# santiagolmedo/gnn_qot_estimation

Measured on AMD Instinct MI355X. Metric: graphs/sec (train step) on 100-node/400-edge synthetic topologies, batch=1024, higher is better.
Workload: dtype f32; 1 GPU; configs[1]: 2-layer TopologicalGNN (TransformerConv+NNConv) hidden=64, 100-node/400-directed-edge topologies, batch=1024 graphs per GPU, dropout 0.5, SGD momentum 0.9, SmoothL1; CSR build included in every step; graphs_per_gpu=1024, global_batch=1024, distinct_graphs_per_gpu=1024, launch=hip-graph replay, 4 whole steps (fwd+bwd+optimizer each) per graph, steps_per_graph=4, collective_in_graph=False, parallelism=dp1, prime_steps=45, collective_world_size=1, all_reduce_floats=68715

## Files before the change

gnn_qot_estimation_amd/_lib.py:

```python
from __future__ import annotations

import ctypes as C
import os
import subprocess

import torch

_HERE = os.path.dirname(os.path.abspath(__file__))
LIB_PATH = os.environ.get("QOT_LIB_PATH") or os.path.join(_HERE, "libqot_gnn.so")
CSRC_DIR = os.path.join(_HERE, "csrc")

_p = C.c_void_p
_i64 = C.c_int64
_int = C.c_int
_f = C.c_float
_u64 = C.c_uint64
_sz = C.c_size_t

ABI_VERSION = 13

_INFER_COMMON = ([_p] * 5 + [_i64] * 3 + [_int, _int, _p, _int, _p, _int, _p, _int] + [_p] * 9
                 + [_f, _f, _p, _int, _int, _int, _p])
_LP_COMMON = ([_p] * 6 + [_i64] * 4 + [_p] * 4 + [_f] + [_p] * 4 + [_f] + [_p] * 4 + [_f, _p, _p] + [_int] * 5 + [_p])

# ... 122 lines not shown
                                      _i64, _i64, _i64, _i64, _i64, _p, _p, _p, _p, _p, _p, _p, _p, _p]),
    "qot_shard_stage_gather": (_int, [_p, _i64, _p, _p, _p, _p, _i64, _i64, _i64, _p, _p, _int, _p, _p, _int, _p, _int, _i64,
                                      _i64, _i64, _i64, _i64, _i64, _p, _p, _p, _p, _p, _p, _p, _p, _p]),
    "qot_gather3": (_int, [_p, _i64, _p, _i64, _p, _p, _p, _i64, _p]),
    "qot_gemm_nt": (_int, [_p, _i64, _p, _i64, _p, _i64, _i64, _int, _int, _p, _p, _p, _p]),
    "qot_gemm_nt_planes": (_int, [_p, _i64, _p, _i64, _p, _i64, _int, _int, _int, _p]),
    "qot_gemm_tn_splits": (_int, [_int, _int, _i64]),
    "qot_gemm256_takes": (_int, [_i64, _int]),
    "qot_gemm_tn_planes": (_int, [_p, _i64, _p, _i64, _p, _int, _int, _i64, _int, _p, _p, _p]),
    "qot_skinny_linear_fwd": (_int, [_p, _p, _p, _i64, _int, _int, _p]),
    "qot_skinny_linear_fwd_logits": (_int, [_p, _p, _p, _i64, _int, _int, _p, _p, _p, _p, _p]),
    "qot_gemm_nt_logits": (_int, [_p, _i64, _p, _i64, _p, _i64, _i64, _int, _int, _p, _p, _p, _p, _p, _p, _p, _p]),
    "qot_skinny_linear_dw_blocks": (_int, [_i64]),
    "qot_skinny_linear_dw": (_int, [_p, _p, _p, _i64, _int, _int, _p]),
    "qot_run_roles": (_int, [_p, _int, _p]),
    "qot_rows_gather": (_int, [_p, _p, _p, _i64, _int, _p]),
    "qot_rows_scatter": (_int, [_p, _p, _p, _i64, _int, _p]),
    **{f"qot_topological_infer{k}_supported": (_int, [_int] * 5) for k in ("", "_mc", "_grad", "_whatif")},
    **{f"qot_topological_infer{k}_max_edges": (_int, [_int] * 3) for k in ("", "_mc", "_grad", "_whatif")},
    "qot_topological_infer": (_int, _INFER_COMMON + [_p]),
    "qot_topological_infer_mc": (_int, _INFER_COMMON + [_int, _i64, _u64, _f, _f, _int, _p]),
    "qot_topological_infer_grad": (_int, _INFER_COMMON + [_p, _int, _p, _p, _p]),
    "qot_topological_infer_whatif": (_int, _INFER_COMMON + [_p, _p, _p, _i64, _p, _p, _i64, _p, _i64, _int, _p]),
    "qot_lightpath_infer": (_int, _LP_COMMON + [_p]),
    "qot_lightpath_infer_grad": (_int, _LP_COMMON + [_p, _int, _p, _p, _p, _p, _p]),
    "qot_lightpath_infer_whatif": (_int, _LP_COMMON + [_p, _p, _p, _i64, _p, _p, _i64, _i64, _p]),
    "qot_status_graph_scratch_bytes": (_sz, [_i64, _i64, _i64, _int]),
    "qot_status_graph_count": (_int, [_p, _p, _p, _i64, _i64, _int, _i64, _i64, _int, _int, _int, C.c_double, _int, _p, _sz, _p,
                                      _p]),
    "qot_status_graph_fill": (_int, [_p, _p, _p, _i64, _i64, _int, _i64, _i64, _int, _int, _int, _int, _p, _int, _p, _int, _p,
                                     _p, _p, _p, _i64, _i64, _p, _p, _p, _p, _p]),
}

MAX_ROLES = 12
(ROLE_CSR_BY_GRAPH, ROLE_TABLE_PROJECT_FWD, ROLE_GATHER3, ROLE_SUM_ROWS, ROLE_NNCONV_FINALIZE64, ROLE_TABLE_PROJECT_BWD,
 ROLE_TABLE_SCORES, ROLE_TABLE_PROJECT_BWD_SCORES) = range(1, 9)


class Role(C.Structure):
    _fields_ = [("kind", C.c_int32), ("reserved", C.c_int32), ("p", C.c_void_p * 18), ("i", C.c_int64 * 8)]


def make_role(kind: int, ptrs, ints) -> Role:
    r = Role()
    r.kind = kind
    for k, t in enumerate(ptrs):
        r.p[k] = None if t is None else (t.data_ptr() if isinstance(t, torch.Tensor) else int(t))
    for k, v in enumerate(ints):
        r.i[k] = int(v)
    return r


def run_roles(roles, stream_handle=None):
    if not roles:
        return
    if len(roles) > MAX_ROLES:
        for k in range(0, len(roles), MAX_ROLES):
            run_roles(roles[k:k + MAX_ROLES], stream_handle)
        return
    arr = (Role * len(roles))(*roles)
    code = (_lib or load()).qot_run_roles(C.addressof(arr), len(roles), stream() if stream_handle is None else stream_handle)
    if code != 0:
        check(code, "qot_run_roles")


_lib = None


class QotError(RuntimeError):
    """A libqot_gnn entry point returned a non-zero status."""


def build_library(verbose: bool = False) -> str:
    cmd = ["make", "-C", CSRC_DIR, "-j", str(min(8, os.cpu_count() or 1))]
    res = subprocess.run(cmd, capture_output=True, text=True)
    if res.returncode != 0:
        raise RuntimeError("building libqot_gnn.so failed:\n" + res.stdout[-4000:] + res.stderr[-8000:])
    if verbose:
# ... 19 lines not shown
        raise QotError(f"libqot_gnn ABI version {lib.qot_abi_version()} != {ABI_VERSION} expected by this package: "
                       "rebuild with `make -C gnn_qot_estimation_amd/csrc`")
    _lib = lib
    return lib


def ptr(t):
    return None if t is None else t.data_ptr()


_raw_stream = getattr(torch._C, "_cuda_getCurrentRawStream", None)
_raw_device = getattr(torch._C, "_cuda_getDevice", None)


def stream():
    if _raw_stream is not None and _raw_device is not None:
        return _raw_stream(_raw_device())
    return torch.cuda.current_stream().cuda_stream


def check(code: int, what: str):
    if code != 0:
        msg = load().qot_error_string(code).decode()
        raise QotError(f"{what} failed with status {code}: {msg}")


def call(name: str, *args):
    if any(isinstance(a, torch.Tensor) for a in args):
        raw = tuple(a.data_ptr() if isinstance(a, torch.Tensor) else a for a in args)
    else:
        raw = args
    code = getattr(_lib or load(), name)(*raw, stream())
    if code != 0:
# ... 2 lines not shown
```

gnn_qot_estimation_amd/csrc/mfma_tile.hpp:

```cpp
#pragma once
#include "common.hpp"

namespace qot {

typedef float f32x16 __attribute__((ext_vector_type(16)));

__device__ __forceinline__ int at4_slot(int g, int hi, int i) { return (2 * g + hi) * 32 + (i ^ (g & 7)); }

__device__ __forceinline__ void store_fragment_grouped(float4* At4, int g, int i, float4 v0, float4 v1) {
    const float4 even = make_float4(v0.x, v0.z, v1.x, v1.z), odd = make_float4(v0.y, v0.w, v1.y, v1.w);
    At4[at4_slot(g, 0, i)] = even;
    At4[at4_slot(g, 1, i)] = odd;
}

__host__ __device__ constexpr int acc_row(int r, int hi) { return (r & 3) + 8 * (r >> 2) + 4 * hi; }

__device__ __forceinline__ f32x16 mfma4(float4 a, float4 b, f32x16 c) {
    c = __builtin_amdgcn_mfma_f32_32x32x2f32(a.x, b.x, c, 0, 0, 0);
    c = __builtin_amdgcn_mfma_f32_32x32x2f32(a.y, b.y, c, 0, 0, 0);
    c = __builtin_amdgcn_mfma_f32_32x32x2f32(a.z, b.z, c, 0, 0, 0);
    c = __builtin_amdgcn_mfma_f32_32x32x2f32(a.w, b.w, c, 0, 0, 0);
    return c;
}

// ... 43 lines not shown
}

template <bool AFFINE>
__device__ __forceinline__ float4 affine_relu4(float4 v, float4 s, float4 t) {
    if (!AFFINE) return v;
    return make_float4(fmaxf(fmaf(v.x, s.x, t.x), 0.f), fmaxf(fmaf(v.y, s.y, t.y), 0.f),
                       fmaxf(fmaf(v.z, s.z, t.z), 0.f), fmaxf(fmaf(v.w, s.w, t.w), 0.f));
}

__device__ __forceinline__ void lds_barrier() {
    asm volatile("s_waitcnt lgkmcnt(0)" ::: "memory");
    __builtin_amdgcn_s_barrier();
    asm volatile("" ::: "memory");
}

__device__ __forceinline__ int64_t xcd_tile(int64_t it, int64_t ntiles) {
    const int nx = 8;
    if ((int)gridDim.x % nx != 0) {
        const int64_t t = (int64_t)blockIdx.x + it * gridDim.x;
        return t < ntiles ? t : -1;
    }
    const int xcd = blockIdx.x % nx, slot = blockIdx.x / nx, per_x = gridDim.x / nx;
    const int64_t chunk = (ntiles + nx - 1) / nx;
    const int64_t local = slot + it * per_x;
    const int64_t t = xcd * chunk + local;
    return (local < chunk && t < ntiles) ? t : -1;
}

}

// ... 12 lines not shown
```

gnn_qot_estimation_amd/csrc/nnconv_finalize_dev.hpp:

```cpp
#pragma once
#include "common.hpp"

namespace qot {

constexpr int kAdjBlocksPerCu = 1;

__device__ __forceinline__ void nnconv_bwd_finalize64_body(const float* __restrict__ slabs, int nslabs, int64_t elems,
                                                           float* __restrict__ dst, int K, int nb1,
                                                           const float* __restrict__ hpart, int hblk, int hn, int KD,
                                                           float* __restrict__ gw1, float* __restrict__ gb1, int vb) {
    if (vb >= nb1) {
        const int t = (vb - nb1) * 4 + (threadIdx.x >> 6);
        if (t >= hn) return;
        const float s = wave_sum_partials(hpart, hblk, hn, t);
        if ((threadIdx.x & 63) == 0) { if (t < KD) gw1[t] = s; else gb1[t - KD] = s; }
        return;
    }
    const int64_t gt = vb * (int64_t)256 + threadIdx.x;
    const int64_t t = gt >> 4;
    const int sub = (int)(gt & 15);
    const bool live = t * 4 < elems;
    float4 acc = f4zero();
    if (live) {
        int sidx = sub;
        for (; sidx + 7 * 16 < nslabs; sidx += 8 * 16) {
            float4 v[8];
#pragma unroll
            for (int u = 0; u < 8; ++u) v[u] = ld4(slabs + (int64_t)(sidx + 16 * u) * elems + 4 * t);
#pragma unroll
            for (int u = 0; u < 8; ++u) acc = add4(acc, v[u]);
        }
        for (; sidx < nslabs; sidx += 16) acc = add4(acc, ld4(slabs + (int64_t)sidx * elems + 4 * t));
// ... 6 lines not shown
    if (!live || sub) return;
    const int64_t e = 4 * t;
    const int a0 = (int)(e & 63), o_ = (int)((e >> 6) & 63), kb = (int)(e >> 12);
    const float v[4] = {acc.x, acc.y, acc.z, acc.w};
#pragma unroll
    for (int c = 0; c < 4; ++c) {
        const int a = a0 + c;
        int64_t idx;
        if (kb < K) idx = ((int64_t)a * 64 + o_) * K + kb;
        else if (kb == K) idx = (int64_t)4096 * K + a * 64 + o_;
        else idx = (int64_t)4096 * (K + 1) + o_ * 64 + a;
        dst[idx] = v[c];
    }
}

}
```

gnn_qot_estimation_amd/csrc/nnconv_gradh64.hip:

```cpp
#include "common.hpp"
#include "mfma_tile.hpp"
#include "split_bf16.hpp"

namespace qot {

constexpr int kGaLd = 516;

constexpr int kGhCap = 256;


template <int D, bool SPLIT = false, bool PRESPLIT = false>
__global__ __launch_bounds__(256, 2) void nnconv_gradh64_kernel(
    const float* __restrict__ g, int ldg, const float* __restrict__ x, int ldx, const float* __restrict__ ea,
    const float* __restrict__ w1, const float* __restrict__ b1, const int32_t* __restrict__ rowptr,
    const int32_t* __restrict__ col, const int32_t* __restrict__ eidx, const float* __restrict__ invdeg,
    const float* __restrict__ Bp, float* __restrict__ partials, int64_t N, const u32x4* __restrict__ Bs = nullptr,
    int64_t bs_planes = 0) {
    constexpr int K = 2 * D;
    static_assert(K <= 8, "one k per lane of the 8-lane group");
    constexpr int NB = K * 2;
    constexpr int NBW = NB / 4;
    constexpr int EPG = kGhCap / 32;
    constexpr int EPF = 5;
    static_assert(SPLIT || !PRESPLIT, "the planes are the split form's");
    __shared__ __attribute__((aligned(16))) float Gt[PRESPLIT ? 3 * kGhPlLd * 4 : 8 * 2 * 32 * 4];
    __shared__ __attribute__((aligned(16))) float GAt[32 * (K * 64 + 4)];
    __shared__ int sj[kGhCap], sr[kGhCap];
    __shared__ __attribute__((aligned(16))) float sea_own[PRESPLIT ? 4 : kGhCap * D];
    static_assert(!PRESPLIT || kGhCap * D <= 3 * kGhPlLd * 4, "sea fits the planes");
    float* const sea = PRESPLIT ? Gt : sea_own;
    __shared__ int rp_l[36];
    constexpr int LDGA = K * 64 + 4;
    float4* Gt4 = reinterpret_cast<float4*>(Gt);
    const int lane = threadIdx.x & 63, wave = threadIdx.x >> 6;
    const int r31 = lane & 31, hi = lane >> 5;
    const int sub = threadIdx.x & 7, il = threadIdx.x >> 3;
    const int c0 = 8 * sub;
    const int64_t ntiles = (N + 31) / 32;

    float wrow[D], brow, aw[D], ab = 0.f;
    brow = (sub < K) ? b1[sub] : 0.f;
#pragma unroll
    for (int d = 0; d < D; ++d) { wrow[d] = (sub < K) ? w1[sub * D + d] : 0.f; aw[d] = 0.f; }

    auto edge = [&](int r, const float4& x0, const float4& x1, const float (&ee)[D]) {
        float pd[8];
#pragma unroll
        for (int k = 0; k < 8; ++k) {
// ... 25 lines not shown
        }
        const float keep = (sub & 1) ? t2[1] : t2[0];
        const float send = (sub & 1) ? t2[0] : t2[1];
        const float tot = keep + dpp_move<0xB1>(send);
        float pre = brow;
#pragma unroll
        for (int d = 0; d < D; ++d) pre = fmaf(wrow[d], ee[d], pre);
        const float gh = (pre > 0.f && sub < K) ? tot : 0.f;
        ab += gh;
#pragma unroll
        for (int d = 0; d < D; ++d) aw[d] = fmaf(gh, ee[d], aw[d]);
    };

#pragma unroll 1
    for (int64_t it = 0;; ++it) {
        const int64_t tile = xcd_tile(it, ntiles);
        if (tile < 0) break;
        const int64_t tile0 = tile * 32;
        const int64_t i = tile0 + il;
        const int64_t tend = (tile0 + 32 < N) ? tile0 + 32 : N;
        constexpr int SL = 3;
        float4 bf[2][8];
        Bf3 bsp[SL + 1];
        const u32x4* bsw = Bs + (int64_t)(wave * NBW) * 4 * 64 + lane;
        if constexpr (SPLIT) {
#pragma unroll
            for (int s = 0; s < SL; ++s) bsp[s] = load_split_b(bsw + s * 64, bs_planes);
        } else {
            const float4* bp = reinterpret_cast<const float4*>(Bp) + (int64_t)(wave * NBW) * 8 * 64 + lane;
#pragma unroll
            for (int gq = 0; gq < 8; ++gq) bf[0][gq] = bp[gq * 64];
// ... 130 lines not shown
    if (threadIdx.x < (D + 1) * 8) {
        const int s8 = threadIdx.x & 7, d = threadIdx.x >> 3;
        float sum = 0.f;
        for (int g32 = 0; g32 < 32; ++g32) sum += red[(d * 32 + g32) * 8 + s8];
        if (s8 < K) partials[(int64_t)blockIdx.x * (K * (D + 1)) + (d < D ? s8 * D + d : K * D + s8)] = sum;
    }
}

}

using namespace qot;

int qot_nnconv_gradh64_launch(const float* grad_out, int ld_g, const float* x, int ld_x, const float* edge_attr, const float* w1,
                              const float* b1, const int32_t* rowptr, const int32_t* col, const int32_t* eid, const float* invdeg,
                              const float* b_perm, const void* b_split, int64_t split_stride, float* workspace, int64_t N, int D,
                              int grid, hipStream_t stream) {
    if (b_split) {
        const char* sar_env = getenv("QOT_GRADH_SPLIT_AFTER_READ");
        const bool presplit = !(sar_env && sar_env[0] == '1' && sar_env[1] == '\0');
        QOT_DISPATCH_D(D, {
            if (kD <= 4) {
                if (presplit)
                    nnconv_gradh64_kernel<(kD <= 4 ? kD : 4), true, true><<<grid, 256, 0, stream>>>(
                        grad_out, ld_g, x, ld_x, edge_attr, w1, b1, rowptr, col, eid, invdeg, nullptr, workspace, N,
                        static_cast<const u32x4*>(b_split), split_stride / 8);
                else
                    nnconv_gradh64_kernel<(kD <= 4 ? kD : 4), true><<<grid, 256, 0, stream>>>(
                        grad_out, ld_g, x, ld_x, edge_attr, w1, b1, rowptr, col, eid, invdeg, nullptr, workspace, N,
                        static_cast<const u32x4*>(b_split), split_stride / 8);
            }
        });
        QOT_LAUNCH_CHECK();
        return QOT_OK;
    }
    QOT_DISPATCH_D(D, {
        if (kD <= 4)
            nnconv_gradh64_kernel<(kD <= 4 ? kD : 4)><<<grid, 256, 0, stream>>>(
                grad_out, ld_g, x, ld_x, edge_attr, w1, b1, rowptr, col, eid, invdeg, b_perm, workspace, N);
    });
    QOT_LAUNCH_CHECK();
    return QOT_OK;
}
```

gnn_qot_estimation_amd/csrc/nnconv_mfma.hip:

```cpp
#include "common.hpp"
#include "mfma_tile.hpp"
#include "nnconv_finalize_dev.hpp"
#include "split_bf16.hpp"

namespace qot {

template <int D, bool TRANSPOSE, bool PRESPLIT = false>
__device__ __forceinline__ void nnconv_gather_tile(
    float* __restrict__ At, const float* __restrict__ x, int ldx, const float* __restrict__ ea,
    const float* __restrict__ w1, const float* __restrict__ b1, const int32_t* __restrict__ rowptr,
    const int32_t* __restrict__ col, const int32_t* __restrict__ eidx, const float* __restrict__ invdeg,
    int64_t tile0, int64_t N, float4& root0, float4& root1, float4* park0 = nullptr, float4* park1 = nullptr) {
    constexpr int K = 2 * D;
    const int sub = threadIdx.x & 7, il = threadIdx.x >> 3;
    const int c0 = 8 * sub;
    const int64_t i = tile0 + il;
    float4 acc0[K + 1], acc1[K + 1];
    root0 = f4zero(); root1 = f4zero();
    int beg = 0, end = 0;
    float srow = 0.f;
    if (i < N) {
        beg = rowptr[i]; end = rowptr[i + 1];
        if (!TRANSPOSE) srow = invdeg[i];
        root0 = ld4(x + i * ldx + c0);
// ... 648 lines not shown
                    x, ld_x, edge_attr, w1, b1, rowptr, col, edge_ids, invdeg, nullptr, bias, out, N, ap,
                    static_cast<const u32x4*>(w_split), split_stride / 8);
            else
                nnconv_mfma64_kernel<(kD <= 4 ? kD : 4), false, true><<<grid, 256, 0, (hipStream_t)stream>>>(
                    x, ld_x, edge_attr, w1, b1, rowptr, col, edge_ids, invdeg, nullptr, bias, out, N, ap,
                    static_cast<const u32x4*>(w_split), split_stride / 8);
        }
    });
    QOT_LAUNCH_CHECK();
    return QOT_OK;
}

int qot_nnconv_gradh64_launch(const float* grad_out, int ld_g, const float* x, int ld_x, const float* edge_attr, const float* w1,
                              const float* b1, const int32_t* rowptr, const int32_t* col, const int32_t* eid, const float* invdeg,
                              const float* b_perm, const void* b_split, int64_t split_stride, float* workspace, int64_t N, int D,
                              int grid, hipStream_t stream);
extern "C" size_t qot_nnconv_gradh_workspace_floats(int D) {
    return (size_t)2 * 256 * 2 * (size_t)(2 * D * (D + 1));
}

static int nnconv_gradh_impl(const float* grad_out, int ld_g, const float* x, int ld_x,
                             const float* edge_attr, const float* w1, const float* b1,
                             const int32_t* rowptr, const int32_t* col, const int32_t* eid,
                             const float* invdeg, const float* b_perm, const void* b_split, int64_t split_stride,
                             float* gw1, float* gb1,
                             float* workspace, int64_t N, int H, int D, qot_stream_t stream_) {
    hipStream_t stream = (hipStream_t)stream_;
    if (N < 0 || !rowptr) return QOT_ERR_BADARG;
    if ((H != 16 && H != 32 && H != 64 && H != 128 && H != 256) || D > 4) return QOT_ERR_UNSUPPORTED;
    if (!grad_out || !x || !w1 || !b1 || !invdeg || !(b_perm || b_split) || (!gw1 != !gb1) || !workspace || (ld_g & 3) ||
        (ld_x & 3) || ((uintptr_t)b_split & 15) || (b_split && ((split_stride & 7) || split_stride < (int64_t)2 * D * 64 * 64)))
        return QOT_ERR_BADARG;
    if (b_split && H != 64) return QOT_ERR_UNSUPPORTED;
    if (!gw1 && H != 64) return QOT_ERR_UNSUPPORTED;
    if (H != 64)
        return qot_nnconv_gradh_gen_launch(grad_out, ld_g, x, ld_x, edge_attr, w1, b1, rowptr, col, eid, invdeg, b_perm,
                                           gw1, gb1, workspace, N, H, D, stream);
    int grid = grid_for(N > 0 ? N : 1, 32);
    if (grid > 2 * num_cus()) grid = 2 * num_cus();
    const int K = 2 * D;
    const int rc = qot_nnconv_gradh64_launch(grad_out, ld_g, x, ld_x, edge_attr, w1, b1, rowptr, col, eid, invdeg, b_perm,
                                             b_split, split_stride, workspace, N, D, grid, stream);
    if (rc != QOT_OK) return rc;
    QOT_LAUNCH_CHECK();
    if (!gw1) return QOT_OK;
    const int n = K * (D + 1);
    gradh_partial_sum_kernel<<<grid_for(n, 4), 256, 0, stream>>>(workspace, grid, n, K * D, gw1, gb1);
    QOT_LAUNCH_CHECK();
    return QOT_OK;
}

extern "C" int qot_nnconv_gradh_fused(const float* grad_out, int ld_g, const float* x, int ld_x,
                                      const float* edge_attr, const float* w1, const float* b1,
                                      const int32_t* rowptr, const int32_t* col, const int32_t* eid,
                                      const float* invdeg, const float* b_perm, float* gw1, float* gb1,
                                      float* workspace, int64_t N, int H, int D, qot_stream_t stream) {
    return nnconv_gradh_impl(grad_out, ld_g, x, ld_x, edge_attr, w1, b1, rowptr, col, eid, invdeg, b_perm, nullptr, 0, gw1, gb1,
// ... 75 lines not shown
```

gnn_qot_estimation_amd/csrc/roles.hip:

```cpp
#include <cstdlib>
#include "common.hpp"
#include "graph_prep_dev.hpp"
#include "mfma_tile.hpp"
#include "nnconv_finalize_dev.hpp"
#include "reduce_dev.hpp"
#include "small_dev.hpp"
#include "tconv_graph_dev.hpp"

namespace qot {

struct RoleTable {
    int n;
    int first[QOT_MAX_ROLES + 1];
    qot_role_t role[QOT_MAX_ROLES];
};

template <typename T>
__device__ __forceinline__ T* rp(const qot_role_t& r, int k) { return reinterpret_cast<T*>(const_cast<void*>(r.p[k])); }

#define QOT_ROLE_H(H, ...)                                            \
    switch (H) {                                                      \
        case 16:  { constexpr int kH = 16;  __VA_ARGS__; } break;     \
        case 32:  { constexpr int kH = 32;  __VA_ARGS__; } break;     \
        case 64:  { constexpr int kH = 64;  __VA_ARGS__; } break;     \
// ... 34 lines not shown
    }
    case QOT_ROLE_GATHER3:
        gather3_body(rp<const float>(ro, 0), (int)ro.i[0], rp<const float>(ro, 1), (int)ro.i[1], rp<const float>(ro, 2),
                     rp<const int32_t>(ro, 3), rp<float>(ro, 4), ro.i[2], (int64_t)vb, rp<const int32_t>(ro, 5),
                     rp<uint16_t>(ro, 6), ro.i[3]);
        break;
    case QOT_ROLE_SUM_ROWS:
        sum_rows_body(rp<const float>(ro, 0), rp<float>(ro, 1), ro.i[0], ro.i[1], ro.i[2], (int)ro.i[3], vb,
                      reinterpret_cast<float*>(dyn_lds));
        break;
    case QOT_ROLE_NNCONV_FINALIZE64:
        nnconv_bwd_finalize64_body(rp<const float>(ro, 0), (int)ro.i[2], ro.i[3], rp<float>(ro, 2), (int)ro.i[4], (int)ro.i[5],
                                   rp<const float>(ro, 1), (int)ro.i[6], (int)ro.i[7], (int)ro.i[4] * (int)ro.i[1],
                                   rp<float>(ro, 3), rp<float>(ro, 4), vb);
        break;
    case QOT_ROLE_TABLE_PROJECT_BWD: {
        const Proj4 p{{rp<const float>(ro, 2), rp<const float>(ro, 3), rp<const float>(ro, 4), rp<const float>(ro, 5)},
                      {nullptr, nullptr, nullptr, nullptr}};
        QOT_ROLE_H((int)ro.i[1], table_project_bwd_body<kH, 1>(rp<const float>(ro, 0), rp<const float>(ro, 1), p, rp<float>(ro, 6),
                                                               rp<float>(ro, 7), rp<float>(ro, 8), (int)ro.i[0], vb,
                                                               reinterpret_cast<float*>(dyn_lds)));
        break;
    }
    case QOT_ROLE_TABLE_SCORES:
        QOT_ROLE_H((int)ro.i[1], table_scores_body<kH>(rp<const float>(ro, 0), rp<const float>(ro, 1), rp<const float>(ro, 2),
                                                       rp<const float>(ro, 3), rp<const float>(ro, 4), rp<const float>(ro, 5),
                                                       rp<float>(ro, 6), rp<float>(ro, 7), (int)ro.i[0], (int)ro.i[2], vb,
                                                       reinterpret_cast<float*>(dyn_lds)));
        break;
    case QOT_ROLE_TABLE_PROJECT_BWD_SCORES: {
// ... 71 lines not shown
        const int64_t nblk = i[0], n = i[1];
        int64_t per = i[2];
        if (nblk <= 0 || n <= 0 || per < 0 || !p[0] || !p[1]) return QOT_ERR_BADARG;
        if (per == 0 || per > nblk) per = nblk;
        i[2] = per;
        const int64_t groups = (nblk + per - 1) / per;
        const bool v4 = (n % 4 == 0) && ((uintptr_t)p[0] % 16 == 0) && ((uintptr_t)p[1] % 16 == 0);
        i[3] = v4 ? 1 : 0;
        const int64_t cols = v4 ? n / 4 : n;
        i[4] = (cols + kSumCols - 1) / kSumCols;
        *blocks = i[4] * groups;
        *lds = (size_t)256 * 16;
        if (*blocks > 0x7fffffff) return QOT_ERR_UNSUPPORTED;
        return QOT_OK;
    }
    case QOT_ROLE_NNCONV_FINALIZE64: {
        const int64_t N = i[0], D = i[1];
        if (N <= 0 || D < 1) return QOT_ERR_BADARG;
        if (D > 4) return QOT_ERR_UNSUPPORTED;
        for (int k = 0; k < 5; ++k) if (!p[k]) return QOT_ERR_BADARG;
        int64_t agrid = (N + 31) / 32;
        if (agrid > (int64_t)num_cus() * kAdjBlocksPerCu) agrid = (int64_t)num_cus() * kAdjBlocksPerCu;
        int64_t hgrid = (N + 31) / 32;
        if (hgrid > 2 * (int64_t)num_cus()) hgrid = 2 * (int64_t)num_cus();
        const int64_t K = 2 * D;
        const int64_t elems = (K + 2) * 64 * 64;
        const int64_t nb1 = (elems / 4 * 16 + 255) / 256;
        const int64_t hn = K * (D + 1);
        i[2] = agrid; i[3] = elems; i[4] = K; i[5] = nb1; i[6] = hgrid; i[7] = hn;
        *blocks = nb1 + (hn + 3) / 4;
        return QOT_OK;
    }
    case QOT_ROLE_TABLE_PROJECT_BWD: {
        const int64_t V = i[0], H = i[1];
        if (V <= 0) return QOT_ERR_BADARG;
        if (!width_ok(H)) return QOT_ERR_UNSUPPORTED;
        for (int k = 0; k < 9; ++k) if (!p[k]) return QOT_ERR_BADARG;
        const int R = table_rows_per_block(V);
        *blocks = 4 * H / R + (V + R - 1) / R;
        *lds = (size_t)(512 * R + R * 4 * H) * 4;
        return QOT_OK;
    }
    case QOT_ROLE_TABLE_SCORES: {
        const int64_t n = i[0], H = i[1], D = i[2];
        if (n <= 0 || D <= 0) return QOT_ERR_BADARG;
// ... 95 lines not shown
        if (total > 0x7fffffff) return QOT_ERR_UNSUPPORTED;
        if (need > lds) lds = need;
    }
    if (n_light == 0) return QOT_OK;
    t.n = n_light;
    for (int r = n_light; r <= QOT_MAX_ROLES; ++r) t.first[r] = (int)total;
    {
        static size_t allowed[kMaxDevices];
        const int lrc = ensure_dyn_lds(reinterpret_cast<const void*>(roles_kernel), lds, allowed);
        if (lrc != QOT_OK) return lrc;
    }
    roles_kernel<<<(int)total, 256, lds, stream>>>(t);
    QOT_LAUNCH_CHECK();
    return QOT_OK;
}
```

gnn_qot_estimation_amd/functional.py:

```python
from __future__ import annotations

import os
from typing import Optional

import torch

from . import _lib, launch_group as LG
from .graph import GraphIndex, require_cuda

P = _lib.ptr


def _f32c(t: torch.Tensor) -> torch.Tensor:
    if t.dtype != torch.float32:
        raise TypeError("the HIP path computes in fp32; got %s" % t.dtype)
    return t.contiguous()


def _off(t: torch.Tensor, floats: int) -> int:
    return t.data_ptr() + 4 * floats


class EmbedFn(torch.autograd.Function):

# ... 879 lines not shown
        gw1, gb1 = gw1f.view(K, D), gb1f.view(K)
        wsh = torch.empty(_lib.load().qot_nnconv_gradh_workspace_floats(D), dtype=torch.float32, device=dev)
        gpar = torch.empty((K + 2) * hh, dtype=torch.float32, device=dev)
        gradh_args = (P(g), hout, P(x), hin, P(edge_attr), P(w1), P(b1), P(graph.rowptr), P(graph.col), P(graph.eid),
                      P(graph.invdeg))
        if split is not None:
            gradh_fn, gradh_args = "qot_nnconv_gradh_split", gradh_args + (P(split[ctx.n_wcat:]), split.numel() // 3)
        else:
            gradh_fn, gradh_args = "qot_nnconv_gradh_fused", gradh_args + (P(bp),)
        if hin == 64 and not os.environ.get("QOT_SPLIT_NNCONV_BWD"):
            gx = torch.empty(N, hin, dtype=torch.float32, device=dev)
            ws = torch.empty(_lib.load().qot_nnconv_adjoint_dw_workspace_floats(D), dtype=torch.float32, device=dev)
            deferred = LG.can_defer(*ctx.receivers)
            _lib.call("qot_nnconv_adjoint_dw", P(g), hout, P(x), hin, P(edge_attr), P(w1), P(b1), P(graph.rowptr_t),
                      P(graph.col_t), P(graph.eid_t), P(graph.invdeg), P(wp_adj), P(gx), P(gpar), 2, P(ws), N, hin, D)
            _lib.call(gradh_fn, *gradh_args, None, None, P(wsh), N, hin, D)
            if deferred:
                LG.defer(_lib.ROLE_NNCONV_FINALIZE64, (ws, wsh, gpar, gw1f, gb1f), (N, D), stage=1)
            else:
                _lib.call("qot_nnconv_bwd_finalize", P(ws), P(wsh), P(gpar), P(gw1f), P(gb1f), N, hin, D)
        else:
            gx = None
            if ctx.needs_input_grad[0]:
                gx = torch.empty(N, hin, dtype=torch.float32, device=dev)
                _lib.call("qot_nnconv_fused", P(g), hout, P(edge_attr), P(w1), P(b1), P(graph.rowptr_t),
                          P(graph.col_t), P(graph.eid_t), P(graph.invdeg), 1, P(wp_adj), None, P(gx), N, hout, D,
                          0, 0.0, 0.0, 0, None)
            ws = torch.empty(_lib.load().qot_nnconv_dw_workspace_floats(N, hin, D), dtype=torch.float32, device=dev)
            _lib.call("qot_nnconv_dw", P(x), hin, P(g), hout, P(edge_attr), P(w1), P(b1), P(graph.rowptr), P(graph.col),
                      P(graph.eid), P(graph.invdeg), P(gpar), P(ws), N, hin, D)
            _lib.call(gradh_fn, *gradh_args, P(gw1), P(gb1), P(wsh), N, hin, D)
        gw2, gb2, gwroot = gpar[:hh * K].view(hh, K), gpar[hh * K:hh * (K + 1)], gpar[hh * (K + 1):].view(hout, hin)
        return gx, gea, gw1, gb1, gw2, gb2, gwroot, gbias, None, None, None, None


# ... 634 lines not shown
```

gnn_qot_estimation_amd/launch_group.py:

```python
from __future__ import annotations

import os

import torch

from . import _lib


def enabled() -> bool:
    return os.environ.get("QOT_NO_LAUNCH_GROUPS", "0") != "1"


def can_defer(*receivers) -> bool:
    if not enabled():
        return False
    for t in receivers:
        if t is None:
            continue
        if not isinstance(t, torch.Tensor) or not t.is_leaf or t.grad is not None:
            return False
        if getattr(t, "_backward_hooks", None) or getattr(t, "_post_accumulate_grad_hooks", None) or not t.is_contiguous():
            return False
    ids = [id(t) for t in receivers if t is not None]
    if len(ids) != len(set(ids)):
        return False
# ... 17 lines not shown
        try:
            _lib.run_roles(roles)
        finally:
            self.keep = []
        for fn in post:
            fn()
        for fn in done:
            fn()


class _BackwardQueue:
    def __init__(self):
        self.clear()

    def pending(self) -> bool:
        return bool(self.stages[0] or self.stages[1])

    def clear(self):
        self.stages = ([], [])
        self.keep = []
        self.stream = None
        self.armed = False


_Q = _BackwardQueue()


def _arm():
    q = _Q
    if not q.armed:
        q.clear()
        q.stream = _lib.stream()
        torch.autograd.Variable._execution_engine.queue_callback(flush)
        q.armed = True
    return q


def defer(kind: int, ptrs, ints, stage: int = 1, keep=()):
    q = _arm()
    q.stages[stage - 1].append(_lib.make_role(kind, ptrs, ints))
    q.keep.extend(t for t in ptrs if isinstance(t, torch.Tensor))
    q.keep.extend(keep)


def flush():
    q = _Q
    if not q.pending():
        q.armed = False
        return
    s1, s2 = q.stages
    stream = q.stream
    q.stages = ([], [])
    try:
        _lib.run_roles(s1, stream)
        _lib.run_roles(s2, stream)
    finally:
        q.keep = []
        q.armed = False
        q.stream = None


def drop_stale():
    if _Q.pending() or _Q.armed:
        gid = getattr(torch._C, "_current_graph_task_id", None)
        if gid is not None and gid() != -1:
            return
        _Q.clear()
```

include/qot_gnn.h:

```cpp
#ifndef QOT_GNN_H
#define QOT_GNN_H

#include <stddef.h>
#include <stdint.h>

#ifdef __cplusplus
extern "C" {
#endif

typedef void* qot_stream_t;

#define QOT_ABI_VERSION 13
#define QOT_OK 0
#define QOT_ERR_UNSUPPORTED (-1)
#define QOT_ERR_BADARG (-2)

int qot_abi_version(void);
const char* qot_error_string(int code);

size_t qot_csr_workspace_bytes(int64_t E, int64_t N, int gat_self_loops);
int qot_csr_build(const int64_t* edge_index, int64_t E, int64_t N, int gat_self_loops,
                  int32_t* rowptr, int32_t* col, int32_t* eid, int32_t* row,
                  int32_t* rowptr_t, int32_t* col_t, int32_t* pos_t, int32_t* eid_t, float* invdeg,
                  void* workspace, size_t workspace_bytes, qot_stream_t stream);
// ... 306 lines not shown
int qot_skinny_linear_fwd(const float* x, const float* w, float* out, int64_t N, int F, int C, qot_stream_t stream);
int qot_skinny_linear_fwd_logits(const float* x, const float* w, float* out, int64_t N, int F, int C, const float* att_src,
                                 const float* att_dst, float* a_src, float* a_dst, qot_stream_t stream);
int qot_skinny_linear_dw_blocks(int64_t N);
int qot_skinny_linear_dw(const float* g, const float* x, float* partials, int64_t N, int F, int C, qot_stream_t stream);

#define QOT_MAX_ROLES 12
enum {
    QOT_ROLE_CSR_BY_GRAPH = 1,
    QOT_ROLE_TABLE_PROJECT_FWD = 2,
    QOT_ROLE_GATHER3 = 3,
    QOT_ROLE_SUM_ROWS = 4,
    QOT_ROLE_NNCONV_FINALIZE64 = 5,
    QOT_ROLE_TABLE_PROJECT_BWD = 6,
    QOT_ROLE_TABLE_SCORES = 7,
    QOT_ROLE_TABLE_PROJECT_BWD_SCORES = 8
};
typedef struct qot_role {
    int32_t kind;
    int32_t reserved;
    const void* p[18];
    int64_t i[8];
} qot_role_t;
int qot_run_roles(const qot_role_t* roles, int n_roles, qot_stream_t stream);

int qot_rows_gather(const float* x, const int32_t* idx, float* out, int64_t n_idx, int C,
                    qot_stream_t stream);
int qot_rows_scatter(const float* grad_out, const int32_t* idx, float* grad_x, int64_t n_idx, int C,
                     qot_stream_t stream);

int qot_topological_infer_supported(int n_max, int max_e, int H, int D, int O);
int qot_topological_infer_max_edges(int n_max, int H, int D);
int qot_topological_infer(const int64_t* node_ids, const int64_t* edge_index, const float* edge_attr,
                          const int64_t* node_ptr, const int64_t* edge_ptr, int64_t N, int64_t E, int64_t B, int n_max,
                          int max_e, const float* t4, int ld4, const float* M, int ldm, const float* P, int V,
                          const float* w_edge, const float* w1, const float* b1, const float* wcat, const float* bias2,
                          const float* w0, const float* b0, const float* w3, const float* b3, float slope_conv,
                          float slope_head, float* out, int H, int D, int O, int32_t* status, qot_stream_t stream);

// ... 84 lines not shown
```

Before: 2.540 million graphs/s.

## Host deferred slab and row-sum reductions as tail blocks inside the gradh kernel

Splits the NNConv backward finalize role into separate slab-sum and gradh-sum roles. Independent reductions (sum_rows, slab sums) can now ride as extra tail blocks on the nnconv_gradh64 launch, with their parameters passed through the kernel argument segment. The gradh kernel call itself is deferred into the launch-group flush so these reductions overlap with it and fewer kernel launches run per step. The cost is extra kernel arguments, more complex flush ordering, and tail blocks that may compete with the main tiles for CUs.

```diff
diff --git a/gnn_qot_estimation_amd/_lib.py b/gnn_qot_estimation_amd/_lib.py
--- a/gnn_qot_estimation_amd/_lib.py
+++ b/gnn_qot_estimation_amd/_lib.py
@@ -160,6 +160,7 @@
     "qot_skinny_linear_dw_blocks": (_int, [_i64]),
     "qot_skinny_linear_dw": (_int, [_p, _p, _p, _i64, _int, _int, _p]),
     "qot_run_roles": (_int, [_p, _int, _p]),
+    "qot_nnconv_gradh_host_roles": (_int, [_p, _int]),
     "qot_rows_gather": (_int, [_p, _p, _p, _i64, _int, _p]),
     "qot_rows_scatter": (_int, [_p, _p, _p, _i64, _int, _p]),
     **{f"qot_topological_infer{k}_supported": (_int, [_int] * 5) for k in ("", "_mc", "_grad", "_whatif")},
@@ -180,7 +181,8 @@
 
 MAX_ROLES = 12
 (ROLE_CSR_BY_GRAPH, ROLE_TABLE_PROJECT_FWD, ROLE_GATHER3, ROLE_SUM_ROWS, ROLE_NNCONV_FINALIZE64, ROLE_TABLE_PROJECT_BWD,
- ROLE_TABLE_SCORES, ROLE_TABLE_PROJECT_BWD_SCORES) = range(1, 9)
+ ROLE_TABLE_SCORES, ROLE_TABLE_PROJECT_BWD_SCORES, ROLE_NNCONV_SLAB_SUM64, ROLE_NNCONV_GRADH_SUM64) = range(1, 11)
+HOSTABLE_ROLES = (ROLE_SUM_ROWS, ROLE_NNCONV_SLAB_SUM64)
 
 
 class Role(C.Structure):
@@ -208,6 +210,13 @@
     code = (_lib or load()).qot_run_roles(C.addressof(arr), len(roles), stream() if stream_handle is None else stream_handle)
     if code != 0:
         check(code, "qot_run_roles")
+
+
+def host_roles(roles):
+    arr = (Role * max(len(roles), 1))(*roles)
+    code = (_lib or load()).qot_nnconv_gradh_host_roles(C.addressof(arr), len(roles))
+    if code != 0:
+        check(code, "qot_nnconv_gradh_host_roles")
 
 
 _lib = None
@@ -257,9 +266,28 @@
 
 
 def stream():
+    if _pinned_stream is not None:
+        return _pinned_stream
     if _raw_stream is not None and _raw_device is not None:
         return _raw_stream(_raw_device())
     return torch.cuda.current_stream().cuda_stream
+
+
+_pinned_stream = None
+
+
+class on_stream:
+
+    def __init__(self, handle):
+        self.handle = handle
+
+    def __enter__(self):
+        global _pinned_stream
+        self.prev, _pinned_stream = _pinned_stream, self.handle
+
+    def __exit__(self, *exc):
+        global _pinned_stream
+        _pinned_stream = self.prev
 
 
 def check(code: int, what: str):
diff --git a/gnn_qot_estimation_amd/csrc/mfma_tile.hpp b/gnn_qot_estimation_amd/csrc/mfma_tile.hpp
--- a/gnn_qot_estimation_amd/csrc/mfma_tile.hpp
+++ b/gnn_qot_estimation_amd/csrc/mfma_tile.hpp
@@ -81,6 +81,18 @@
     asm volatile("" ::: "memory");
 }
 
+__device__ __forceinline__ int64_t xcd_tile(int64_t it, int64_t ntiles, unsigned grid) {
+    const int nx = 8;
+    if ((int)grid % nx != 0) {
+        const int64_t t = (int64_t)blockIdx.x + it * grid;
+        return t < ntiles ? t : -1;
+    }
+    const int xcd = blockIdx.x % nx, slot = blockIdx.x / nx, per_x = grid / nx;
+    const int64_t chunk = (ntiles + nx - 1) / nx;
+    const int64_t local = slot + it * per_x;
+    const int64_t t = xcd * chunk + local;
+    return (local < chunk && t < ntiles) ? t : -1;
+}
 __device__ __forceinline__ int64_t xcd_tile(int64_t it, int64_t ntiles) {
     const int nx = 8;
     if ((int)gridDim.x % nx != 0) {
diff --git a/gnn_qot_estimation_amd/csrc/nnconv_finalize_dev.hpp b/gnn_qot_estimation_amd/csrc/nnconv_finalize_dev.hpp
--- a/gnn_qot_estimation_amd/csrc/nnconv_finalize_dev.hpp
+++ b/gnn_qot_estimation_amd/csrc/nnconv_finalize_dev.hpp
@@ -5,17 +5,16 @@
 
 constexpr int kAdjBlocksPerCu = 1;
 
-__device__ __forceinline__ void nnconv_bwd_finalize64_body(const float* __restrict__ slabs, int nslabs, int64_t elems,
-                                                           float* __restrict__ dst, int K, int nb1,
-                                                           const float* __restrict__ hpart, int hblk, int hn, int KD,
-                                                           float* __restrict__ gw1, float* __restrict__ gb1, int vb) {
-    if (vb >= nb1) {
-        const int t = (vb - nb1) * 4 + (threadIdx.x >> 6);
-        if (t >= hn) return;
-        const float s = wave_sum_partials(hpart, hblk, hn, t);
-        if ((threadIdx.x & 63) == 0) { if (t < KD) gw1[t] = s; else gb1[t - KD] = s; }
-        return;
-    }
+__device__ __forceinline__ void nnconv_gradh_sum64_body(const float* __restrict__ hpart, int hblk, int hn, int KD,
+                                                        float* __restrict__ gw1, float* __restrict__ gb1, int vb) {
+    const int t = vb * 4 + (threadIdx.x >> 6);
+    if (t >= hn) return;
+    const float s = wave_sum_partials(hpart, hblk, hn, t);
+    if ((threadIdx.x & 63) == 0) { if (t < KD) gw1[t] = s; else gb1[t - KD] = s; }
+}
+
+__device__ __forceinline__ void nnconv_slab_sum64_body(const float* __restrict__ slabs, int nslabs, int64_t elems,
+                                                       float* __restrict__ dst, int K, int vb) {
     const int64_t gt = vb * (int64_t)256 + threadIdx.x;
     const int64_t t = gt >> 4;
     const int sub = (int)(gt & 15);
@@ -52,4 +51,26 @@
     }
 }
 
+__device__ __forceinline__ void nnconv_bwd_finalize64_body(const float* __restrict__ slabs, int nslabs, int64_t elems,
+                                                           float* __restrict__ dst, int K, int nb1,
+                                                           const float* __restrict__ hpart, int hblk, int hn, int KD,
+                                                           float* __restrict__ gw1, float* __restrict__ gb1, int vb) {
+    if (vb >= nb1) nnconv_gradh_sum64_body(hpart, hblk, hn, KD, gw1, gb1, vb - nb1);
+    else nnconv_slab_sum64_body(slabs, nslabs, elems, dst, K, vb);
 }
+
+constexpr int kHostedSumRows = 1;
+constexpr int kHostedSlabSum64 = 2;
+struct HostedJob {
+    int32_t kind, flag;
+    const float* src;
+    float* dst;
+    int64_t a, b, c;
+};
+struct HostedTable {
+    int n;
+    int first[QOT_MAX_ROLES + 1];
+    HostedJob job[QOT_MAX_ROLES];
+};
+
+}
diff --git a/gnn_qot_estimation_amd/csrc/nnconv_gradh64.hip b/gnn_qot_estimation_amd/csrc/nnconv_gradh64.hip
--- a/gnn_qot_estimation_amd/csrc/nnconv_gradh64.hip
+++ b/gnn_qot_estimation_amd/csrc/nnconv_gradh64.hip
@@ -1,5 +1,7 @@
 #include "common.hpp"
 #include "mfma_tile.hpp"
+#include "nnconv_finalize_dev.hpp"
+#include "reduce_dev.hpp"
 #include "split_bf16.hpp"
 
 namespace qot {
@@ -8,9 +10,18 @@
 
 constexpr int kGhCap = 256;
 
+__device__ __forceinline__ void gradh_hosted_tail(const HostedTable& t, int vt, float* __restrict__ scratch) {
+    int r = 0;
+    while (r + 1 < t.n && vt >= t.first[r + 1]) ++r;
+    const HostedJob& jb = t.job[r];
+    const int vb = vt - t.first[r];
+    if (jb.kind == kHostedSumRows) sum_rows_body(jb.src, jb.dst, jb.a, jb.b, jb.c, jb.flag, vb, scratch);
+    else if (jb.kind == kHostedSlabSum64) nnconv_slab_sum64_body(jb.src, (int)jb.a, jb.b, jb.dst, jb.flag, vb);
+}
 
 template <int D, bool SPLIT = false, bool PRESPLIT = false>
 __global__ __launch_bounds__(256, 2) void nnconv_gradh64_kernel(
+    const HostedTable hosted_by_value, int n_main,
     const float* __restrict__ g, int ldg, const float* __restrict__ x, int ldx, const float* __restrict__ ea,
     const float* __restrict__ w1, const float* __restrict__ b1, const int32_t* __restrict__ rowptr,
     const int32_t* __restrict__ col, const int32_t* __restrict__ eidx, const float* __restrict__ invdeg,
@@ -32,6 +43,15 @@
     __shared__ int rp_l[36];
     constexpr int LDGA = K * 64 + 4;
     float4* Gt4 = reinterpret_cast<float4*>(Gt);
+    if ((int)blockIdx.x >= n_main) {
+#if defined(__HIP_DEVICE_COMPILE__)
+        typedef const HostedTable __attribute__((address_space(4))) * KernargTable;
+        gradh_hosted_tail(*(const HostedTable*)(KernargTable)__builtin_amdgcn_kernarg_segment_ptr(), (int)blockIdx.x - n_main, GAt);
+#else
+        gradh_hosted_tail(hosted_by_value, (int)blockIdx.x - n_main, GAt);
+#endif
+        return;
+    }
     const int lane = threadIdx.x & 63, wave = threadIdx.x >> 6;
     const int r31 = lane & 31, hi = lane >> 5;
     const int sub = threadIdx.x & 7, il = threadIdx.x >> 3;
@@ -87,7 +107,7 @@
 
 #pragma unroll 1
     for (int64_t it = 0;; ++it) {
-        const int64_t tile = xcd_tile(it, ntiles);
+        const int64_t tile = xcd_tile(it, ntiles, (unsigned)n_main);
         if (tile < 0) break;
         const int64_t tile0 = tile * 32;
         const int64_t i = tile0 + il;
@@ -248,7 +268,9 @@
 int qot_nnconv_gradh64_launch(const float* grad_out, int ld_g, const float* x, int ld_x, const float* edge_attr, const float* w1,
                               const float* b1, const int32_t* rowptr, const int32_t* col, const int32_t* eid, const float* invdeg,
                               const float* b_perm, const void* b_split, int64_t split_stride, float* workspace, int64_t N, int D,
-                              int grid, hipStream_t stream) {
+                              int grid, const qot::HostedTable& hosted, hipStream_t stream) {
+    const int n_main = grid;
+    grid += hosted.n > 0 ? hosted.first[hosted.n] : 0;
     if (b_split) {
         const char* sar_env = getenv("QOT_GRADH_SPLIT_AFTER_READ");
         const bool presplit = !(sar_env && sar_env[0] == '1' && sar_env[1] == '\0');
@@ -256,11 +278,11 @@
             if (kD <= 4) {
                 if (presplit)
                     nnconv_gradh64_kernel<(kD <= 4 ? kD : 4), true, true><<<grid, 256, 0, stream>>>(
-                        grad_out, ld_g, x, ld_x, edge_attr, w1, b1, rowptr, col, eid, invdeg, nullptr, workspace, N,
+                        hosted, n_main, grad_out, ld_g, x, ld_x, edge_attr, w1, b1, rowptr, col, eid, invdeg, nullptr, workspace, N,
                         static_cast<const u32x4*>(b_split), split_stride / 8);
                 else
                     nnconv_gradh64_kernel<(kD <= 4 ? kD : 4), true><<<grid, 256, 0, stream>>>(
-                        grad_out, ld_g, x, ld_x, edge_attr, w1, b1, rowptr, col, eid, invdeg, nullptr, workspace, N,
+                        hosted, n_main, grad_out, ld_g, x, ld_x, edge_attr, w1, b1, rowptr, col, eid, invdeg, nullptr, workspace, N,
                         static_cast<const u32x4*>(b_split), split_stride / 8);
             }
         });
@@ -270,7 +292,7 @@
     QOT_DISPATCH_D(D, {
         if (kD <= 4)
             nnconv_gradh64_kernel<(kD <= 4 ? kD : 4)><<<grid, 256, 0, stream>>>(
-                grad_out, ld_g, x, ld_x, edge_attr, w1, b1, rowptr, col, eid, invdeg, b_perm, workspace, N);
+                hosted, n_main, grad_out, ld_g, x, ld_x, edge_attr, w1, b1, rowptr, col, eid, invdeg, b_perm, workspace, N);
     });
     QOT_LAUNCH_CHECK();
     return QOT_OK;
diff --git a/gnn_qot_estimation_amd/csrc/nnconv_mfma.hip b/gnn_qot_estimation_amd/csrc/nnconv_mfma.hip
--- a/gnn_qot_estimation_amd/csrc/nnconv_mfma.hip
+++ b/gnn_qot_estimation_amd/csrc/nnconv_mfma.hip
@@ -686,7 +686,8 @@
 int qot_nnconv_gradh64_launch(const float* grad_out, int ld_g, const float* x, int ld_x, const float* edge_attr, const float* w1,
                               const float* b1, const int32_t* rowptr, const int32_t* col, const int32_t* eid, const float* invdeg,
                               const float* b_perm, const void* b_split, int64_t split_stride, float* workspace, int64_t N, int D,
-                              int grid, hipStream_t stream);
+                              int grid, const qot::HostedTable& hosted, hipStream_t stream);
+int qot_hosted_take(qot::HostedTable* t, qot_role_t* planned);
 extern "C" size_t qot_nnconv_gradh_workspace_floats(int D) {
     return (size_t)2 * 256 * 2 * (size_t)(2 * D * (D + 1));
 }
@@ -698,6 +699,9 @@
                              float* gw1, float* gb1,
                              float* workspace, int64_t N, int H, int D, qot_stream_t stream_) {
     hipStream_t stream = (hipStream_t)stream_;
+    HostedTable hosted;
+    qot_role_t hosted_roles[QOT_MAX_ROLES];
+    const int n_hosted = qot_hosted_take(&hosted, hosted_roles);
     if (N < 0 || !rowptr) return QOT_ERR_BADARG;
     if ((H != 16 && H != 32 && H != 64 && H != 128 && H != 256) || D > 4) return QOT_ERR_UNSUPPORTED;
     if (!grad_out || !x || !w1 || !b1 || !invdeg || !(b_perm || b_split) || (!gw1 != !gb1) || !workspace || (ld_g & 3) ||
@@ -705,14 +709,21 @@
         return QOT_ERR_BADARG;
     if (b_split && H != 64) return QOT_ERR_UNSUPPORTED;
     if (!gw1 && H != 64) return QOT_ERR_UNSUPPORTED;
-    if (H != 64)
-        return qot_nnconv_gradh_gen_launch(grad_out, ld_g, x, ld_x, edge_attr, w1, b1, rowptr, col, eid, invdeg, b_perm,
-                                           gw1, gb1, workspace, N, H, D, stream);
+    for (int r = 0; r < n_hosted; ++r) {
+        const uintptr_t src = (uintptr_t)hosted.job[r].src, w0 = (uintptr_t)workspace;
+        if (src >= w0 && src < w0 + qot_nnconv_gradh_workspace_floats(D) * sizeof(float)) return QOT_ERR_BADARG;
+    }
+    if (H != 64) {
+        const int rc = qot_nnconv_gradh_gen_launch(grad_out, ld_g, x, ld_x, edge_attr, w1, b1, rowptr, col, eid, invdeg, b_perm,
+                                                   gw1, gb1, workspace, N, H, D, stream);
+        if (rc != QOT_OK || n_hosted == 0) return rc;
+        return qot_run_roles(hosted_roles, n_hosted, stream_);
+    }
     int grid = grid_for(N > 0 ? N : 1, 32);
     if (grid > 2 * num_cus()) grid = 2 * num_cus();
     const int K = 2 * D;
     const int rc = qot_nnconv_gradh64_launch(grad_out, ld_g, x, ld_x, edge_attr, w1, b1, rowptr, col, eid, invdeg, b_perm,
-                                             b_split, split_stride, workspace, N, D, grid, stream);
+                                             b_split, split_stride, workspace, N, D, grid, hosted, stream);
     if (rc != QOT_OK) return rc;
     QOT_LAUNCH_CHECK();
     if (!gw1) return QOT_OK;
diff --git a/gnn_qot_estimation_amd/csrc/roles.hip b/gnn_qot_estimation_amd/csrc/roles.hip
--- a/gnn_qot_estimation_amd/csrc/roles.hip
+++ b/gnn_qot_estimation_amd/csrc/roles.hip
@@ -72,6 +72,13 @@
                                    rp<const float>(ro, 1), (int)ro.i[6], (int)ro.i[7], (int)ro.i[4] * (int)ro.i[1],
                                    rp<float>(ro, 3), rp<float>(ro, 4), vb);
         break;
+    case QOT_ROLE_NNCONV_SLAB_SUM64:
+        nnconv_slab_sum64_body(rp<const float>(ro, 0), (int)ro.i[2], ro.i[3], rp<float>(ro, 2), (int)ro.i[4], vb);
+        break;
+    case QOT_ROLE_NNCONV_GRADH_SUM64:
+        nnconv_gradh_sum64_body(rp<const float>(ro, 1), (int)ro.i[6], (int)ro.i[7], (int)ro.i[4] * (int)ro.i[1], rp<float>(ro, 3),
+                                rp<float>(ro, 4), vb);
+        break;
     case QOT_ROLE_TABLE_PROJECT_BWD: {
         const Proj4 p{{rp<const float>(ro, 2), rp<const float>(ro, 3), rp<const float>(ro, 4), rp<const float>(ro, 5)},
                       {nullptr, nullptr, nullptr, nullptr}};
@@ -173,11 +180,15 @@
         if (*blocks > 0x7fffffff) return QOT_ERR_UNSUPPORTED;
         return QOT_OK;
     }
-    case QOT_ROLE_NNCONV_FINALIZE64: {
+    case QOT_ROLE_NNCONV_FINALIZE64:
+    case QOT_ROLE_NNCONV_SLAB_SUM64:
+    case QOT_ROLE_NNCONV_GRADH_SUM64: {
         const int64_t N = i[0], D = i[1];
+        const bool slab = r.kind != QOT_ROLE_NNCONV_GRADH_SUM64, gh = r.kind != QOT_ROLE_NNCONV_SLAB_SUM64;
         if (N <= 0 || D < 1) return QOT_ERR_BADARG;
         if (D > 4) return QOT_ERR_UNSUPPORTED;
-        for (int k = 0; k < 5; ++k) if (!p[k]) return QOT_ERR_BADARG;
+        if (slab && (!p[0] || !p[2])) return QOT_ERR_BADARG;
+        if (gh && (!p[1] || !p[3] || !p[4])) return QOT_ERR_BADARG;
         int64_t agrid = (N + 31) / 32;
         if (agrid > (int64_t)num_cus() * kAdjBlocksPerCu) agrid = (int64_t)num_cus() * kAdjBlocksPerCu;
         int64_t hgrid = (N + 31) / 32;
@@ -187,7 +198,7 @@
         const int64_t nb1 = (elems / 4 * 16 + 255) / 256;
         const int64_t hn = K * (D + 1);
         i[2] = agrid; i[3] = elems; i[4] = K; i[5] = nb1; i[6] = hgrid; i[7] = hn;
-        *blocks = nb1 + (hn + 3) / 4;
+        *blocks = (slab ? nb1 : 0) + (gh ? (hn + 3) / 4 : 0);
         return QOT_OK;
     }
     case QOT_ROLE_TABLE_PROJECT_BWD: {
@@ -313,3 +324,57 @@
     QOT_LAUNCH_CHECK();
     return QOT_OK;
 }
+
+namespace {
+struct HostedState {
+    int n = 0;
+    qot_role_t role[QOT_MAX_ROLES];
+    int64_t blocks[QOT_MAX_ROLES];
+};
+thread_local HostedState g_hosted;
+}
+
+extern "C" int qot_nnconv_gradh_host_roles(const qot_role_t* roles, int n_roles) {
+    if (n_roles < 0 || n_roles > QOT_MAX_ROLES || (n_roles > 0 && !roles)) return QOT_ERR_BADARG;
+    HostedState st;
+    int64_t total = 0;
+    for (int r = 0; r < n_roles; ++r) {
+        st.role[r] = roles[r];
+        if (st.role[r].kind != QOT_ROLE_SUM_ROWS && st.role[r].kind != QOT_ROLE_NNCONV_SLAB_SUM64)
+            return st.role[r].kind >= QOT_ROLE_CSR_BY_GRAPH && st.role[r].kind <= QOT_ROLE_NNCONV_GRADH_SUM64 ? QOT_ERR_UNSUPPORTED
+                                                                                                               : QOT_ERR_BADARG;
+        size_t need;
+        const int rc = plan_role(st.role[r], &st.blocks[r], &need);
+        if (rc != QOT_OK) return rc;
+        total += st.blocks[r];
+        if (total > 0x3fffffff) return QOT_ERR_UNSUPPORTED;
+    }
+    st.n = n_roles;
+    g_hosted = st;
+    return QOT_OK;
+}
+
+int qot_hosted_take(qot::HostedTable* t, qot_role_t* planned) {
+    HostedState& st = g_hosted;
+    const int n = st.n;
+    t->n = n;
+    int total = 0;
+    for (int r = 0; r < n; ++r) {
+        const qot_role_t& ro = st.role[r];
+        planned[r] = ro;
+        HostedJob& jb = t->job[r];
+        t->first[r] = total;
+        total += (int)st.blocks[r];
+        if (ro.kind == QOT_ROLE_SUM_ROWS) {
+            jb = HostedJob{kHostedSumRows, (int32_t)ro.i[3], (const float*)ro.p[0], (float*)const_cast<void*>(ro.p[1]), ro.i[0],
+                           ro.i[1], ro.i[2]};
+        } else {
+            jb = HostedJob{kHostedSlabSum64, (int32_t)ro.i[4], (const float*)ro.p[0], (float*)const_cast<void*>(ro.p[2]), ro.i[2],
+                           ro.i[3], 0};
+        }
+    }
+    for (int r = n; r <= QOT_MAX_ROLES; ++r) t->first[r] = total;
+    for (int r = n; r < QOT_MAX_ROLES; ++r) t->job[r] = HostedJob{0, 0, nullptr, nullptr, 0, 0, 0};
+    st.n = 0;
+    return n;
+}
diff --git a/gnn_qot_estimation_amd/functional.py b/gnn_qot_estimation_amd/functional.py
--- a/gnn_qot_estimation_amd/functional.py
+++ b/gnn_qot_estimation_amd/functional.py
@@ -917,11 +917,17 @@
             deferred = LG.can_defer(*ctx.receivers)
             _lib.call("qot_nnconv_adjoint_dw", P(g), hout, P(x), hin, P(edge_attr), P(w1), P(b1), P(graph.rowptr_t),
                       P(graph.col_t), P(graph.eid_t), P(graph.invdeg), P(wp_adj), P(gx), P(gpar), 2, P(ws), N, hin, D)
-            _lib.call(gradh_fn, *gradh_args, None, None, P(wsh), N, hin, D)
-            if deferred:
-                LG.defer(_lib.ROLE_NNCONV_FINALIZE64, (ws, wsh, gpar, gw1f, gb1f), (N, D), stage=1)
+            if deferred and LG.hosted_sums():
+                LG.defer(_lib.ROLE_NNCONV_SLAB_SUM64, (ws, None, gpar), (N, D), stage=1)
+                LG.defer_gradh(gradh_fn, gradh_args + (None, None, P(wsh), N, hin, D),
+                               (_lib.ROLE_NNCONV_GRADH_SUM64, (None, wsh, None, gw1f, gb1f), (N, D)),
+                               keep=(g, x, edge_attr, w1, b1, graph, split, bp))
             else:
-                _lib.call("qot_nnconv_bwd_finalize", P(ws), P(wsh), P(gpar), P(gw1f), P(gb1f), N, hin, D)
+                _lib.call(gradh_fn, *gradh_args, None, None, P(wsh), N, hin, D)
+                if deferred:
+                    LG.defer(_lib.ROLE_NNCONV_FINALIZE64, (ws, wsh, gpar, gw1f, gb1f), (N, D), stage=1)
+                else:
+                    _lib.call("qot_nnconv_bwd_finalize", P(ws), P(wsh), P(gpar), P(gw1f), P(gb1f), N, hin, D)
         else:
             gx = None
             if ctx.needs_input_grad[0]:
diff --git a/gnn_qot_estimation_amd/launch_group.py b/gnn_qot_estimation_amd/launch_group.py
--- a/gnn_qot_estimation_amd/launch_group.py
+++ b/gnn_qot_estimation_amd/launch_group.py
@@ -9,6 +9,10 @@
 
 def enabled() -> bool:
     return os.environ.get("QOT_NO_LAUNCH_GROUPS", "0") != "1"
+
+
+def hosted_sums() -> bool:
+    return os.environ.get("QOT_NO_HOSTED_SUMS", "0") != "1"
 
 
 def can_defer(*receivers) -> bool:
@@ -56,10 +60,11 @@
         self.clear()
 
     def pending(self) -> bool:
-        return bool(self.stages[0] or self.stages[1])
+        return bool(self.stages[0] or self.stages[1] or self.gradh)
 
     def clear(self):
         self.stages = ([], [])
+        self.gradh = []
         self.keep = []
         self.stream = None
         self.armed = False
@@ -85,17 +90,59 @@
     q.keep.extend(keep)
 
 
+def _take_hostable(s1):
+    hosted, rest = [], []
+    for r in s1:
+        (hosted if r.kind in _lib.HOSTABLE_ROLES and len(hosted) < _lib.MAX_ROLES else rest).append(r)
+    return hosted, rest
+
+
+def defer_gradh(fn: str, args, partial_sum, keep=()):
+    q = _arm()
+    q.keep.extend(keep)
+    q.keep.extend(t for t in partial_sum[1] if isinstance(t, torch.Tensor))
+    role = _lib.make_role(*partial_sum)
+    if os.environ.get("QOT_HOSTED_SUMS_EARLY", "0") == "1":
+        hosted, q.stages[0][:] = _take_hostable(q.stages[0])
+        _lib.host_roles(hosted)
+        with _lib.on_stream(q.stream):
+            _lib.call(fn, *args)
+        q.stages[0].append(role)
+    else:
+        q.gradh.append((fn, args, role))
+
+
+def plan(s1, s2, gradh):
+    if not gradh:
+        return [("roles", r) for r in (s1, s2) if r]
+    hosted, rest = _take_hostable(s1)
+    out = [("gradh", fn, args, hosted if k == 0 else []) for k, (fn, args, _) in enumerate(gradh)]
+    sums = [role for _, _, role in gradh]
+    if rest:
+        out += [("roles", rest + sums)] + ([("roles", s2)] if s2 else [])
+    else:
+        out.append(("roles", s2 + sums))
+    return out
+
+
 def flush():
     q = _Q
     if not q.pending():
         q.armed = False
         return
     s1, s2 = q.stages
-    stream = q.stream
-    q.stages = ([], [])
+    gradh, stream = q.gradh, q.stream
+    q.stages, q.gradh = ([], []), []
     try:
-        _lib.run_roles(s1, stream)
-        _lib.run_roles(s2, stream)
+        for step in plan(s1, s2, gradh):
+            if step[0] == "gradh":
+                _, fn, args, hosted = step
+                if hosted:
+                    _lib.host_roles(hosted)
+                with _lib.on_stream(stream):
+                    _lib.call(fn, *args)
+            else:
+                _lib.run_roles(step[1], stream)
     finally:
         q.keep = []
         q.armed = False
diff --git a/include/qot_gnn.h b/include/qot_gnn.h
--- a/include/qot_gnn.h
+++ b/include/qot_gnn.h
@@ -344,7 +344,9 @@
     QOT_ROLE_NNCONV_FINALIZE64 = 5,
     QOT_ROLE_TABLE_PROJECT_BWD = 6,
     QOT_ROLE_TABLE_SCORES = 7,
-    QOT_ROLE_TABLE_PROJECT_BWD_SCORES = 8
+    QOT_ROLE_TABLE_PROJECT_BWD_SCORES = 8,
+    QOT_ROLE_NNCONV_SLAB_SUM64 = 9,
+    QOT_ROLE_NNCONV_GRADH_SUM64 = 10
 };
 typedef struct qot_role {
     int32_t kind;
@@ -353,6 +355,8 @@
     int64_t i[8];
 } qot_role_t;
 int qot_run_roles(const qot_role_t* roles, int n_roles, qot_stream_t stream);
+
+int qot_nnconv_gradh_host_roles(const qot_role_t* roles, int n_roles);
 
 int qot_rows_gather(const float* x, const int32_t* idx, float* out, int64_t n_idx, int C,
                     qot_stream_t stream);
```

After: 2.584 million graphs/s (median of 6 runs). 1.7% higher.
